# DerekGloudemans/3D-playground

Measured on AMD Instinct MI355X. Metric: training images/sec at 1920x1080, ResNet-50 3D-RetinaNet, higher is better.
Workload: dtype f32; 1 GPU; resnet50 directional 3D-RetinaNet, 1920x1080 synthetic frames, batch 8 per GPU, 10 GT boxes/image, fp32, fwd+loss+bwd+clip+Adam (BASELINE configs[1]); global_batch=8, parallelism=dp1

## Files before the change

3d-playground_amd/retinanet_mi355x/_hip.py:

```python
import ctypes
import os

import torch

_HERE = os.path.dirname(os.path.abspath(__file__))
LIB_PATH = os.environ.get("RN_LIB_PATH") or os.path.join(_HERE, "lib", "libretinanet_mi355x.so")
_lib = None

c_i32, c_i64, c_f32, c_f64, c_vp = ctypes.c_int, ctypes.c_int64, ctypes.c_float, ctypes.c_double, ctypes.c_void_p

SIGNATURES = {
    "rn_version": (ctypes.c_char_p, []),
    "rn_check_device": (c_i32, []),
    "rn_get_fp32_mfma": (c_i32, []),
    "rn_set_fp32_mfma": (c_i32, [c_i32]),
    "rn_get_option": (c_i32, [c_i32]),
    "rn_set_option": (c_i32, [c_i32, c_i32]),
    "rn_fp32_split_min_k": (c_i32, []),
    "rn_split_weights": (c_i32, [c_vp, c_vp, c_i64, c_i32, c_vp]),
    "rn_split_weights_f16": (c_i32, [c_vp, c_vp, c_vp, c_i64, c_i32, c_vp]),
    "rn_amax": (c_i32, [c_vp, c_i64, c_i32, c_vp, c_vp]),
    "rn_stream_capture_id": (c_i32, [c_vp, ctypes.POINTER(ctypes.c_ulonglong)]),
    "rn_anchor_count": (c_i64, [c_i32, c_i32]),
    "rn_anchor_base_boxes": (None, [c_vp]),
# ... 167 lines not shown
    "rn_tile_lists": (c_i32, [c_vp, c_i64, c_vp, c_vp, c_vp, c_vp, c_vp]),
    "rn_wino_input_both_group_lists": (c_i32, [ctypes.POINTER(WinoGroup), c_vp, c_vp, c_i32, c_i64, c_i64, c_vp, c_vp, c_vp, c_vp, c_vp, c_vp]),
    "rn_wino_output_group_flags": (c_i32, [ctypes.POINTER(WinoGroup), c_vp, c_i32, c_i64, c_i64, c_vp, c_vp, c_i32, c_i32, c_i64, c_vp, c_vp, c_vp]),
    "rn_wino_output_group": (c_i32, [ctypes.POINTER(WinoGroup), c_vp, c_i32, c_i64, c_i64, c_vp, c_vp, c_i32, c_i32, c_i64, c_vp]),
    "rn_conv_igemm_grouped": (c_i32, [ctypes.POINTER(ConvGroup), c_vp, c_vp, c_vp, c_vp]),
    "rn_conv_igemm": (c_i32, [ctypes.POINTER(ConvDesc), c_vp, c_vp, c_vp, c_vp, c_vp, c_vp, c_vp, c_vp, c_vp]),
    "rn_conv_splitk_workspace_bytes": (c_i64, [ctypes.POINTER(ConvDesc)]),
    "rn_conv_igemm_wants_f16": (c_i32, [ctypes.POINTER(ConvDesc)]),
    "rn_conv_igemm_splitk": (c_i32, [ctypes.POINTER(ConvDesc)] + [c_vp] * 10),
    "rn_conv_wgrad": (c_i32, [c_vp, c_i32, c_vp, c_vp, c_vp] + [c_i32] * 12 + [c_vp]),
    "rn_pack_weights": (c_i32, [c_vp, c_vp] + [c_i32] * 7 + [c_vp] + [c_i32] * 4 + [c_vp]),
    "rn_unpack_wgrad": (c_i32, [c_vp, c_vp, c_vp] + [c_i32] * 6 + [c_vp] * 7),
    "rn_bn_fold": (c_i32, [c_vp, c_vp, c_vp, c_vp, c_f32, c_i32, c_vp, c_vp, c_vp, c_vp]),
    "rn_nchw_to_nhwc4": (c_i32, [c_vp, c_vp, c_i32, c_i32, c_i32, c_vp, c_vp]),
    "rn_maxpool_fwd": (c_i32, [c_vp, c_vp, c_vp] + [c_i32] * 6 + [c_vp]),
    "rn_maxpool_bwd": (c_i32, [c_vp, c_vp, c_vp, c_vp] + [c_i32] * 7 + [c_vp, c_vp]),
    "rn_colsum": (c_i32, [c_vp, c_i64, c_i32, c_i32, c_vp, c_i32, c_vp, c_vp]),
    "rn_colsum_workspace_bytes": (c_i64, [c_i64, c_i32]),
    "rn_upsample_add_bwd": (c_i32, [c_vp, c_vp] + [c_i32] * 6 + [c_vp, c_vp]),
    "rn_relu_mask": (c_i32, [c_vp, c_vp, c_i64, c_vp]),
    "rn_sigmoid_bwd_pad": (c_i32, [c_vp, c_vp, c_vp, c_i32, c_i64, c_i32, c_i32, c_i64, c_vp, c_vp]),
    "rn_sigmoid_bwd_pad_flags": (c_i32, [c_vp, c_vp, c_vp, c_i32, c_i32, c_i32, c_i32, c_i32, c_i64, c_vp, c_vp, c_vp]),
    "rn_add_inplace": (c_i32, [c_vp, c_vp, c_i64, c_i64, c_vp, c_vp]),
    "rn_wino_input": (c_i32, [c_vp, c_vp, c_i32, c_i32, c_i32, c_i32, c_i64, c_i64, c_vp]),
    "rn_wino_output": (c_i32, [c_vp, c_vp, c_i32, c_i32, c_i32, c_i32, c_i64, c_i64, c_vp, c_vp, c_vp, c_vp, c_i32, c_i32, c_i64, c_vp]),
    "rn_wino_weights": (c_i32, [c_vp, c_vp, c_i32, c_i32, c_i32, c_vp, c_vp]),
    "rn_wino_dy": (c_i32, [c_vp, c_vp, c_i32, c_i32, c_i32, c_i32, c_i64, c_i64, c_vp]),
    "rn_wino_dw": (c_i32, [c_vp, c_vp, c_i32, c_i32, c_vp]),
    "rn_conv_wgrad_batched": (c_i32, [c_vp, c_i32, c_vp, c_vp, c_vp, c_i32, c_i64, c_i64, c_i64, c_i32] + [c_i32] * 12 + [c_vp, c_i32, c_vp, c_i32, c_vp]),
    "rn_conv_wgrad_batched_det": (c_i32, [c_vp, c_i32, c_vp, c_vp, c_vp, c_i32, c_i64, c_i64, c_i64, c_i32] + [c_i32] * 12 + [c_vp, c_i32, c_vp, c_i32, c_vp, c_i64, c_vp]),
    "rn_conv_wgrad_batched_flags": (c_i32, [c_vp, c_i32, c_vp, c_vp, c_vp, c_i32, c_i64, c_i64, c_i64, c_i32] + [c_i32] * 12 + [c_vp, c_i32, c_vp, c_i32, c_vp, c_vp, c_i64, c_vp]),
    "rn_conv_wgrad_det_workspace_bytes": (c_i64, [c_i32, c_i32, c_i64] + [c_i32] * 9),
    "rn_conv_wgrad_plan": (c_i32, [c_i32, c_i32, c_i64, c_i64, c_i64, c_i32] + [c_i32] * 12 + [c_i32, c_i32, c_i32, c_vp]),
    "rn_f32_to_bf16": (c_i32, [c_vp, c_vp, c_i64, c_vp]),
    "rn_bf16_to_f32": (c_i32, [c_vp, c_vp, c_i64, c_vp]),
    "rn_conv_igemm_bf16": (c_i32, [ctypes.POINTER(ConvDesc), c_vp, c_vp, c_vp, c_i32, c_vp, c_vp, c_vp, c_vp, c_vp]),
    "rn_conv_igemm_bf16_grouped": (c_i32, [ctypes.POINTER(ConvGroup), c_vp, c_i32, c_vp, c_vp, c_vp]),
    "rn_conv_igemm_bf16_tile_rows": (c_i32, [ctypes.POINTER(ConvGroup), c_i32]),
    "rn_maxpool_fwd_fp8out": (c_i32, [c_vp, c_vp] + [c_i32] * 6 + [c_f32, c_vp]),
    "rn_conv_igemm_fp8_tile_rows": (c_i32, [ctypes.POINTER(ConvGroup), c_i32]),
    "rn_conv_igemm_fp8_tile": (c_i32, [ctypes.POINTER(ConvDesc), c_i32]),
    "rn_conv_igemm_bf16_tile": (c_i32, [ctypes.POINTER(ConvDesc), c_i32]),
    "rn_fp8_quantize": (c_i32, [c_vp, c_vp, c_i64, c_f32, c_vp]),
    "rn_fp8_dequantize": (c_i32, [c_vp, c_vp, c_i64, c_f32, c_vp]),
    "rn_fp8_to_bf16": (c_i32, [c_vp, c_vp, c_i64, c_f32, c_vp]),
    "rn_bf16_to_fp8": (c_i32, [c_vp, c_vp, c_i64, c_f32, c_vp]),
    "rn_fp8_quantize_rows": (c_i32, [c_vp, c_vp, c_vp, c_i64, c_i32, c_vp]),
    "rn_conv_igemm_fp8": (c_i32, [ctypes.POINTER(ConvDesc), c_vp, c_vp, c_vp, c_i32, c_vp, c_vp, c_vp, c_f32, c_f32, c_vp]),
    "rn_conv_igemm_fp8_grouped": (c_i32, [ctypes.POINTER(ConvGroup), c_vp, c_i32, c_vp, c_vp, c_f32, c_f32, c_vp]),
    "rn_conv_wgrad_bf16": (c_i32, [c_vp, c_i32, c_vp, c_vp, c_vp] + [c_i32] * 11 + [c_vp]),
    "rn_conv_wgrad_bf16_grouped": (c_i32, [c_i32, ctypes.POINTER(c_vp), c_i32, ctypes.POINTER(c_vp), c_vp, c_vp, c_i32,
                                           ctypes.POINTER(c_i32), ctypes.POINTER(c_i32)] + [c_i32] * 6 + [c_vp]),
    "rn_maxpool_fwd_bf16out": (c_i32, [c_vp, c_vp, c_vp] + [c_i32] * 6 + [c_vp]),
    "rn_maxpool_bwd_bf16in": (c_i32, [c_vp, c_vp, c_vp, c_vp] + [c_i32] * 7 + [c_vp]),
    "rn_upsample_add_bwd_bf16": (c_i32, [c_vp, c_vp] + [c_i32] * 6 + [c_vp]),
    "rn_sigmoid_bwd_pad_bf16": (c_i32, [c_vp, c_vp, c_vp, c_i32, c_i64, c_i32, c_i32, c_i64, c_vp]),
    "rn_relu_bf16": (c_i32, [c_vp, c_vp, c_i64, c_vp]),
    "rn_opt_workspace_bytes": (c_i64, [c_i32]),
    "rn_opt_clip_adam": (c_i32, [c_vp, c_vp, c_i32, c_f32, c_f32, c_f32, c_f32, c_f32, c_i32, c_i32, c_vp, c_vp, c_vp]),
    "rn_opt_clip_adam_dev": (c_i32, [c_vp, c_vp, c_i32, c_f32, c_f32, c_f32, c_f32, c_f32, c_vp, c_i32, c_vp, c_vp, c_vp]),
    "rn_opt_clip_adam_hp": (c_i32, [c_vp, c_vp, c_i32, c_vp, c_vp, c_i32, c_vp, c_vp, c_vp]),
})


RN_ERRORS = {10001: "RN_EINVAL (bad size / unsupported shape)",
             10002: "RN_ETOOMANY (more than RN_MAX_GT=256 label rows per image)"}
# ... 51 lines not shown
```

3d-playground_amd/retinanet_mi355x/conv.py:

```python
import ctypes
import os

import torch

from . import _hip, prof

ConvDesc = _hip.ConvDesc

ACT_NONE, ACT_RELU, ACT_SIGMOID = 0, 1, 2


def kpad(kh, kw, c):
    return (kh * kw * c + 31) // 32 * 32


def out_size(n, k, stride, pad):
    return (n + 2 * pad - k) // stride + 1


def pack_weights(weight, mode=0, scale=None, kw_pad=None, c_pad=None, taps=None, presplit=True):
    lib = _hip.load()
    w = _hip.f32c(weight.detach())
    _hip.need_gpu(w, scale)
    cout, cin, kh, kw = w.shape
# ... 653 lines not shown
def dgrad_s2_classes(dy, class_weights, in_hw, cin, k, pad, flops=0.0, **kw):
    N, Ho, Wo, _ = dy.shape
    Hi, Wi = in_hw
    dx = torch.empty((N, Hi, Wi, cin), dtype=torch.float32, device=dy.device)
    classes = s2_classes(k, pad)
    if len(classes) < 4:
        dx.zero_()
    total_taps = sum(c[2][1] * c[2][3] for c in classes)
    slot = amax_slot(dy.device, N) if want_amax() else None
    for (ph, pw, (r0, nr, s0, ns), (dh0, dw0)), wc in zip(classes, class_weights):
        gh, gw = (Hi - ph + 1) // 2, (Wi - pw + 1) // 2
        if gh <= 0 or gw <= 0:
            continue
        conv_igemm(dy, wc, dx, (gh, gw, cin, nr, ns, 1, -1, (dh0, dw0), 0), out_map=(2, ph, pw, Hi, Wi),
                   flops=flops * nr * ns / total_taps, amax=slot, **kw)
    if slot is not None:
        amax_attach(dx, slot)
    return dx


def wgrad(dy, x, dw, cout, k, stride, pad, kw_pad=None, in_relu=False, flops=0.0, colsum=None):
    lib = _hip.load()
    N, Ho, Wo, ldy = dy.shape
    _, Hi, Wi, Cin = x.shape
    kind = "conv_wgrad" + (" %dx%dx%d %d->%d k%d s%d" % (N, Ho, Wo, Cin, cout, k, stride) if prof.BY_SHAPE else "")
    am = (amax_words(dy), amax_words(x)) if want_amax() and dy.is_contiguous() and x.is_contiguous() else (None, None)
    rc = prof.timed(kind, flops, lambda: _wgrad_call(
        lib, dy.device, dy.data_ptr(), ldy, x.data_ptr(), dw.data_ptr(), _hip.ptr(colsum), 1, 0, 0, 0, 0,
        (N, Hi, Wi, Cin, Ho, Wo, cout, k, k if kw_pad is None else kw_pad, stride, pad, int(in_relu)), amax=am))
    _hip.check(rc, "rn_conv_wgrad")
    return dw


def unpack_wgrad(dw, w_packed, weight_shape, kw_pad=None, c_pad=None, scale=None, mean=None, rstd=None, colsum=None,
                 want_bn=False, out=None):
    lib = _hip.load()
    cout, cin, kh, kw = weight_shape
    kw_pad = kw if kw_pad is None else kw_pad
    c_pad = (cin + 3) // 4 * 4 if c_pad is None else c_pad
    if out is not None:
        dweight, dgamma, dbeta = out
        assert tuple(dweight.shape) == tuple(weight_shape) and dweight.is_contiguous() and dweight.dtype == torch.float32
        assert (dgamma is not None) == bool(want_bn) and (dbeta is not None) == (colsum is not None)
    else:
        dweight = torch.empty(weight_shape, dtype=torch.float32, device=dw.device)
        dgamma = torch.empty(cout, dtype=torch.float32, device=dw.device) if want_bn else None
        dbeta = torch.empty(cout, dtype=torch.float32, device=dw.device) if colsum is not None else None
    _hip.check(lib.rn_unpack_wgrad(dw.data_ptr(), _hip.ptr(w_packed), dweight.data_ptr(), cout, cin, kh, kw, kw_pad,
                                   c_pad, _hip.ptr(scale), _hip.ptr(mean), _hip.ptr(rstd), _hip.ptr(colsum),
                                   _hip.ptr(dgamma), _hip.ptr(dbeta), _hip.stream()), "rn_unpack_wgrad")
    return dweight, dgamma, dbeta


def bn_fold(gamma, beta, mean, var, eps=1e-5):
    lib = _hip.load()
    C = gamma.numel()
    out = torch.empty((3, C), dtype=torch.float32, device=gamma.device)
    _hip.check(lib.rn_bn_fold(_hip.f32c(gamma.detach()).data_ptr(), _hip.f32c(beta.detach()).data_ptr(),
                              _hip.f32c(mean).data_ptr(), _hip.f32c(var).data_ptr(), eps, C, out[0].data_ptr(),
                              out[1].data_ptr(), out[2].data_ptr(), _hip.stream()), "rn_bn_fold")
    return out[0], out[1], out[2]


def nchw_to_nhwc4(img):
    lib = _hip.load()
    img = _hip.f32c(img)
# ... 398 lines not shown
```

3d-playground_amd/retinanet_mi355x/engine.py:

```python
import os

import torch

from . import _hip, arch, conv as cv, ops, prof


FUSE_DY = os.environ.get("RN_WINO_FUSE_DY", "1") != "0"
SPARSE_REG = os.environ.get("RN_SPARSE_REG", "1") != "0"
SPARSE_REG_LISTS = os.environ.get("RN_SPARSE_REG_LISTS", "1") != "0"
GROUPED_WGRAD_BF16 = os.environ.get("RN_GROUPED_WGRAD_BF16", "1") != "0"
S2_SHORTCUT_COMPACT = os.environ.get("RN_S2_SHORTCUT_COMPACT", "1") != "0"
STEM_BF16_PRODUCTS = os.environ.get("RN_STEM_BF16_PRODUCTS", "1") != "0"


def _qscale(t):
    return getattr(t, "_rn_scale", None) or getattr(t, "_rn_qscale", None)


def _as_fp8(t):
    if t is None or t.dtype == torch.uint8:
        return t
    q = getattr(t, "_rn_q8", None)
    if q is None:
        sc = _qscale(t)
# ... 311 lines not shown
            return
        for g, x in zip(gs, xs):
            self.bwd_params(g, x)

    def bwd_data(self, g, in_hw, add=None, mask=None, mask_mode=2, add2=None):
        s = self.spec
        if self.bf16:
            assert add2 is None
            kw = dict(add=add, add_mode=1 if add is not None else 0, mask=mask, mask_mode=mask_mode,
                      flops=self.flops(g.shape[0], g.shape[1], g.shape[2]))
            if s.stride == 2 and s.k > 1:
                return cv.dgrad_s2_classes_bf16(g, self.dgrad_weights16(), in_hw, s.cin, s.k, s.pad, **kw)
            if s.stride == 2 and s.k == 1 and s.pad == 0 and mask is None and S2_SHORTCUT_COMPACT:
                Hi, Wi = in_hw
                N, Ho, Wo, _ = g.shape
                if add is None:
                    dx = torch.zeros((N, Hi, Wi, s.cin), dtype=torch.bfloat16, device=g.device)
                else:
                    assert add.shape == (N, Hi, Wi, s.cin) and add.dtype == torch.bfloat16 and add.is_contiguous()
                    dx = add
                return cv.conv_igemm_bf16(g, self.dgrad_weights16(), dx, (Ho, Wo, s.cin, 1, 1, 1, -1, 0, 0), out_map=(2, 0, 0, Hi, Wi),
                                          add=add, add_mode=1 if add is not None else 0, flops=kw["flops"])
            return cv.dgrad_any_bf16(g, self.dgrad_weights16(), in_hw, s.cin, s.k, s.stride, s.pad, **kw)
        if self.wino_active and add2 is None and g.shape[3] == s.cout and g.is_contiguous():
            ready, self.dy_v = getattr(self, "dy_v", None), None
            return cv.wino_conv_group([g], self.wino_weights(1), adds=None if add is None else [add],
                                      masks=None if mask is None else [mask], mask_mode=mask_mode, V_ready=ready)[0]
        kw = dict(add=add, add_mode=1 if add is not None else 0, mask=mask, mask_mode=mask_mode,
                  flops=self.flops(g.shape[0], g.shape[1], g.shape[2]))
        if s.stride == 2 and s.k > 1:
            assert add2 is None
            return cv.dgrad_s2_classes(g, self.dgrad_weights(), in_hw, s.cin, s.k, s.pad, **kw)
        return cv.dgrad(g, self.dgrad_weights(), in_hw, s.cin, s.k, s.stride, s.pad, add2=add2, **kw)

    def bwd_data_compact(self, g):
        s = self.spec
        assert s.k == 1 and s.stride == 2
        N, Ho, Wo, _ = g.shape
        out = torch.empty((N, Ho, Wo, s.cin), dtype=torch.float32, device=g.device)
        return cv.conv_igemm(g, self.dgrad_weights(), out, (Ho, Wo, s.cin, 1, 1, 1, -1, 0, 0), flops=self.flops(N, Ho, Wo))

    def grad_names(self):
        s = self.spec
        if s.bn:
            return [s.name + ".weight", s.bn + ".weight", s.bn + ".bias"]
        return [s.name + ".weight"] + ([s.name + ".bias"] if s.bias else [])

    def finish(self, out=None):
        s = self.spec
        dst = None
        if out is not None:
            names = self.grad_names()
            dst = (out[names[0]], out[names[1]] if s.bn else None, out[names[-1]] if len(names) > 1 else None)
        dweight, dgamma, dbeta = cv.unpack_wgrad(
            self.dw, self.wf, tuple(self.weight.shape), kw_pad=self.kw_pad, c_pad=self.cin_pad, scale=self.scale,
            mean=self.mean, rstd=self.rstd, colsum=self.cs, want_bn=bool(s.bn), out=dst)
        out = {s.name + ".weight": dweight}
        if s.bn:
            out[s.bn + ".weight"] = dgamma
            out[s.bn + ".bias"] = dbeta
        elif s.bias:
            out[s.name + ".bias"] = dbeta
        self.dw = self.cs = self.wd = self.uf = self.ud = self.saved_v = self.dy_v = None
        return out


# ... 567 lines not shown
                main0.wait_stream(ws)
                cv.side_release(ws)
            held.clear()

        def aside(fn, tensors):
            nonlocal wg_count
            ws = wss[wg_count % len(wss)]
            wg_count += 1
            if cv.want_amax():
                for t in tensors:
                    if t.dtype == torch.float32 and t.is_contiguous():
                        cv.amax_words(t)
            ws.wait_event(torch.cuda.current_stream(dreg.device).record_event())
            with torch.cuda.stream(ws):
                fn()
            held.append(tuple(tensors) + tuple(getattr(t, "_rn_amax", (None,))[0] for t in tensors))

        def wg(L, g, x, in_relu=False):
            if wss is None:
                L.bwd_params(g, x, in_relu=in_relu)
            elif L.wino_active and not L.bf16:
                L.bwd_params(g, x, in_relu=in_relu, side=wss[0] if os.environ.get("RN_WGRAD_WINO", "1") != "0" else None)
            else:
                aside(lambda: L.bwd_params(g, x, in_relu=in_relu), (g, x))

        def wg_group(L, gs, xs, wino=False, flags=None, lists=None):
            if wss is None or os.environ.get("RN_WGRAD_TOWERS", "0") == "0":
                L.bwd_params_group(gs, xs, wino=wino, flags=flags, lists=lists)
            elif wino or L.wino_active:
                L.bwd_params_group(gs, xs, wino=wino, side=wss[0], flags=flags, lists=lists)
            else:
                aside(lambda: L.bwd_params_group(gs, xs), tuple(gs) + tuple(xs))

        def done(layer):
            nonlocal next_bucket
            if batched:
                pending.append(layer)
                grads.update({n: views[n] for n in layer.grad_names()})
            else:
                g = layer.finish(views)
                grads.update(g)
                if self.grad_hook is not None:
                    self.grad_hook(g)
            if flat is not None and layer.spec.name == buckets[next_bucket][2]:
                if batched:
                    join()
                    self._unpack_bucket(next_bucket, pending, views)
                    pending.clear()
                if self.bucket_hook is not None:
                    self.bucket_hook(next_bucket, flat[buckets[next_bucket][0]:buckets[next_bucket][1]])
                next_bucket += 1

        ACT = _as_bf16 if self.fp8 else (lambda t: t)
        pyramid, counts = [ACT(t) for t in S["pyramid"]], S["counts"]
        B = dreg.shape[0]
        A = dreg.shape[1]
        dpyr = [None] * 5
        hws = [(f.shape[1], f.shape[2]) for f in pyramid]
        side = self.tower_streams(dreg.device)
        main = torch.cuda.current_stream(dreg.device)
        if side is not None:
            fork = main.record_event()
        retired = []
        for ti, (prefix, dout, width, sig) in enumerate((("regressionModel", dreg, self.n_reg, None),
                                                         ("classificationModel", dcls, self.num_classes, cls))):
            Lout = Ls[prefix + ".output"]
# ... 59 lines not shown
        done(L)
        L = Ls["fpn.P3_1"]
        wg(L, dp3sum, c3)
        dc3 = L.bwd_data(dp3sum, hw(c3))
        done(L)
        L = Ls["fpn.P4_2"]
        wg(L, dp4, p4sum)
        dp4sum = L.bwd_data(dp4, hw(p4sum))
        cv.upsample_add_bwd(dp3sum, dp4sum)
        done(L)
        L = Ls["fpn.P4_1"]
        wg(L, dp4sum, c4)
        dc4 = L.bwd_data(dp4sum, hw(c4))
        done(L)
        L = Ls["fpn.P5_2"]
        wg(L, dp5, p5lat)
        dp5lat = L.bwd_data(dp5, hw(p5lat))
        cv.upsample_add_bwd(dp4sum, dp5lat)
        done(L)
        L = Ls["fpn.P5_1"]
        wg(L, dp5lat, c5)
        dc5 = L.bwd_data(dp5lat, hw(c5), add=dc5, mask=c5)
        done(L)
        lateral = {"layer2": dc3, "layer3": dc4}
        g = dc5
        nblocks = len(self.blocks)
        for bi in range(nblocks - 1, -1, -1):
            pre, roles = self.blocks[bi]
            xin, t1, t2, z = (ACT(t) for t in S["blocks"][bi])
            S["blocks"][bi] = None
            in_hw = hw(xin)
            last = roles["conv2"] if self.kind == "basic" else roles["conv3"]
            tin = t1 if self.kind == "basic" else t2
            wg(last, g, tin)
            gt = last.bwd_data(g, hw(tin), mask=tin)
            done(last)
            if self.kind != "basic":
                wg(roles["conv2"], gt, t1)
                gt = roles["conv2"].bwd_data(gt, hw(t1), mask=t1)
                done(roles["conv2"])
            layer_name = pre.split(".")[0]
            first_of_layer = pre.endswith(".0")
            extra = None
            if first_of_layer and bi > 0:
                prev_layer = self.blocks[bi - 1][0].split(".")[0]
                extra = lateral.get(prev_layer)
            dcompact = None
            if "down" in roles:
                wg(roles["down"], g, xin)
                if roles["down"].spec.stride == 2 and roles["conv1"].spec.stride == 1 and not self.bwd16:
                    dcompact = roles["down"].bwd_data_compact(g)
                    dres = extra
                else:
                    dres = roles["down"].bwd_data(g, in_hw, add=extra)
                done(roles["down"])
            else:
                dres = g if extra is None else cv.add_(extra, g)
            wg(roles["conv1"], gt, xin)
            g = roles["conv1"].bwd_data(gt, in_hw, add=dres, mask=xin if bi > 0 else None, add2=dcompact)
            done(roles["conv1"])
            del layer_name
        gstem = (cv.maxpool_bwd_bf16 if self.bwd16 else cv.maxpool_bwd)(S["stem"], g, S["pool_arg"], relu_mask=True)
        wg(Ls["conv1"], gstem, S["x4"])
        done(Ls["conv1"])
        join()
        assert flat is None or next_bucket == len(buckets), "backward finished layers in an order finish_order() does not describe"
        return grads
```

include/retinanet_mi355x.h:

```cpp
#ifndef RETINANET_MI355X_H
#define RETINANET_MI355X_H

#include <stdint.h>

#ifdef __cplusplus
extern "C" {
#endif

#define RN_OK 0
#define RN_EINVAL 10001
#define RN_ETOOMANY 10002
#define RN_MAX_GT 256
#define RN_LEVELS 5

const char *rn_version(void);
int rn_check_device(void);

int64_t rn_anchor_count(int height, int width);
void rn_anchor_base_boxes(double out[RN_LEVELS * 9 * 4]);
int rn_anchors_fwd(float *out, int height, int width, void *stream);

int rn_pairwise_iou(const float *a, const float *b, float *iou, int64_t A, int N, void *stream);

int64_t rn_focal_workspace_bytes(int B, int64_t A);
// ... 246 lines not shown
typedef struct rn_conv_group {
    int n;
    int tile_end[RN_MAX_GROUP];
    rn_conv_desc d[RN_MAX_GROUP];
    const float *x[RN_MAX_GROUP];
    float *y[RN_MAX_GROUP];
    const float *add[RN_MAX_GROUP];
    const float *mask[RN_MAX_GROUP];
} rn_conv_group;
int rn_conv_igemm_grouped(const rn_conv_group *g, const float *w_packed, const float *scale, const float *shift,
                          void *stream);

int rn_conv_wgrad(const float *dy, int ldy, const float *x, float *dw, float *colsum, int N, int Hi, int Wi,
                  int Cin, int Ho, int Wo, int Cout, int kh, int kw, int stride, int pad, int in_relu, void *stream);
int rn_conv_wgrad_batched(const float *dy, int ldy, const float *x, float *dw, float *colsum, int nbatch,
                          int64_t dy_bstride, int64_t x_bstride, int64_t dw_bstride, int colsum_batch, int N, int Hi, int Wi,
                          int Cin, int Ho, int Wo, int Cout, int kh, int kw, int stride, int pad, int in_relu,
                          const void *dy_amax, int dy_amax_n, const void *x_amax, int x_amax_n, void *stream);
int64_t rn_conv_wgrad_det_workspace_bytes(int ldy, int nbatch, int64_t dw_bstride, int N, int Hi, int Wi, int Cin, int Ho, int Wo,
                                          int Cout, int kh, int kw);
int rn_conv_wgrad_batched_det(const float *dy, int ldy, const float *x, float *dw, float *colsum, int nbatch,
                              int64_t dy_bstride, int64_t x_bstride, int64_t dw_bstride, int colsum_batch, int N, int Hi, int Wi,
                              int Cin, int Ho, int Wo, int Cout, int kh, int kw, int stride, int pad, int in_relu,
                              const void *dy_amax, int dy_amax_n, const void *x_amax, int x_amax_n, void *workspace, int64_t workspace_bytes,
                              void *stream);
int rn_conv_wgrad_batched_flags(const float *dy, int ldy, const float *x, float *dw, float *colsum, int nbatch,
                                int64_t dy_bstride, int64_t x_bstride, int64_t dw_bstride, int colsum_batch, int N, int Hi, int Wi,
                                int Cin, int Ho, int Wo, int Cout, int kh, int kw, int stride, int pad, int in_relu,
                                const void *dy_amax, int dy_amax_n, const void *x_amax, int x_amax_n, const void *k_active,
                                void *workspace, int64_t workspace_bytes, void *stream);
int rn_conv_wgrad_plan(int ldy, int nbatch, int64_t dy_bstride, int64_t x_bstride, int64_t dw_bstride, int colsum_batch, int N, int Hi,
                       int Wi, int Cin, int Ho, int Wo, int Cout, int kh, int kw, int stride, int pad, int in_relu, int have_amax,
                       int have_flags, int det, int32_t *out);

int rn_f32_to_bf16(const float *src, void *dst, int64_t n, void *stream);
int rn_bf16_to_f32(const void *src, float *dst, int64_t n, void *stream);
int rn_conv_igemm_bf16(const rn_conv_desc *d, const void *x, const void *w_packed, void *y, int y_is_f32,
                       const float *scale, const float *shift, const void *add, const void *mask, void *stream);
int rn_conv_igemm_bf16_grouped(const rn_conv_group *g, const void *w_packed, int y_is_f32, const float *scale,
                               const float *shift, void *stream);
int rn_conv_igemm_bf16_tile_rows(const rn_conv_group *g, int y_is_f32);
int rn_fp8_quantize(const float *src, void *dst, int64_t n, float inv_scale, void *stream);
int rn_maxpool_fwd_fp8out(const float *x, void *y, int N, int H, int W, int C, int Ho, int Wo, float inv_scale, void *stream);
int rn_fp8_dequantize(const void *src, float *dst, int64_t n, float scale, void *stream);
int rn_fp8_to_bf16(const void *src, void *dst, int64_t n, float scale, void *stream);
int rn_bf16_to_fp8(const void *src, void *dst, int64_t n, float inv_scale, void *stream);
int rn_fp8_quantize_rows(const float *w_packed, void *w_q, float *row_scale, int64_t rows, int Kpad, void *stream);
int rn_conv_igemm_fp8(const rn_conv_desc *d, const void *x_q, const void *w_q, void *y, int y_is_f32, const float *scale,
                      const float *shift, const void *add_q, float add_scale, float out_inv_scale, void *stream);
int rn_conv_igemm_fp8_tile_rows(const rn_conv_group *g, int y_is_f32);
int rn_conv_igemm_fp8_tile(const rn_conv_desc *d, int y_is_f32);
int rn_conv_igemm_bf16_tile(const rn_conv_desc *d, int y_is_f32);
int rn_conv_igemm_fp8_grouped(const rn_conv_group *g, const void *w_q, int y_is_f32, const float *scale, const float *shift,
                              float add_scale, float out_inv_scale, void *stream);

int rn_conv_wgrad_bf16(const void *dy, int ldy, const void *x, float *dw, float *colsum, int N, int Hi, int Wi, int Cin,
                       int Ho, int Wo, int Cout, int kh, int kw, int stride, int pad, void *stream);
int rn_conv_wgrad_bf16_grouped(int n, const void *const *dy, int ldy, const void *const *x, float *dw, float *colsum, int N,
                               const int *Hi, const int *Wi, int Cin, int Cout, int kh, int kw, int stride, int pad, void *stream);

int rn_maxpool_fwd_bf16out(const float *x, void *y, uint8_t *argmax, int N, int H, int W, int C, int Ho, int Wo, void *stream);
int rn_maxpool_bwd_bf16in(const float *x, const void *dy, const uint8_t *argmax, float *dx, int N, int H, int W, int C, int Ho,
                          int Wo, int relu_mask, void *stream);
int rn_upsample_add_bwd_bf16(const void *src, void *dst, int N, int Hs, int Ws, int Hd, int Wd, int C, void *stream);
int rn_sigmoid_bwd_pad_bf16(const float *dy, const float *s, void *out, int B, int64_t rows_per_image, int C, int ld,
                            int64_t src_batch_stride, void *stream);
// ... 343 lines not shown
```

Baseline: 132.6 images/sec.

## Fuse 1x1 conv weight-gradient and data-gradient into one backward kernel for 64->256

Adds a HIP kernel that computes both dW and dX for 1x1 stride-1 convolutions with Cin=64, Cout=256 in a single pass. Each dy tile is loaded once, split into fp16 hi/lo operands in LDS, and used for both the split-precision MFMA weight-gradient accumulation and the data-gradient product. The kernel also folds in the column sum, the ReLU mask and the amax tracking. This removes the second read of dy and one launch per bottleneck conv3 and downsample layer of that shape. In exchange it accumulates dw with global atomicAdd, so results are non-deterministic; it is gated off in deterministic mode.

```diff
diff --git a/3d-playground_amd/csrc/conv_bwd_1x1.hip b/3d-playground_amd/csrc/conv_bwd_1x1.hip
--- /dev/null
+++ b/3d-playground_amd/csrc/conv_bwd_1x1.hip
@@ -0,0 +1,283 @@
+#include <type_traits>
+
+#include "common.h"
+#include "conv_bwd_1x1_geom.h"
+#include "mfma_split.h"
+
+#if !RN_EXPERIMENT
+#undef RN_BF_KO
+#endif
+#ifndef RN_BF_KO
+#define RN_BF_KO 0
+#endif
+#if !RN_EXPERIMENT
+#undef RN_BF_ND
+#endif
+#ifndef RN_BF_ND
+#define RN_BF_ND 1
+#endif
+
+typedef float f32x16 __attribute__((ext_vector_type(16)));
+typedef float f32x4v __attribute__((ext_vector_type(4)));
+typedef short s16x4w __attribute__((ext_vector_type(4)));
+typedef short s16x8w __attribute__((ext_vector_type(8)));
+
+struct Bwd1x1Args {
+    const float *dy, *x;
+    const char *wd;
+    const float *w_unscale;
+    float *dx, *dw, *colsum;
+    const void *mask;
+    unsigned *sign_out;
+    const void *dy_amax, *x_amax;
+    void *dx_amax;
+    int HW, spi, per;
+};
+
+__device__ __forceinline__ f16x8 bf_tr_operand(const char *img, unsigned a0, unsigned a1) {
+    typedef __attribute__((address_space(3))) s16x4w *lp;
+    const s16x4w lo = __builtin_amdgcn_ds_read_tr16_b64_v4i16((lp)(__attribute__((address_space(3))) char *)(img + a0));
+    const s16x4w hi = __builtin_amdgcn_ds_read_tr16_b64_v4i16((lp)(__attribute__((address_space(3))) char *)(img + a1));
+    const s16x8w v = {lo[0], lo[1], lo[2], lo[3], hi[0], hi[1], hi[2], hi[3]};
+    return __builtin_bit_cast(f16x8, v);
+}
+
+template <int MASK>
+__global__ __launch_bounds__(256, 2) void conv_bwd_1x1_kernel(const Bwd1x1Args p) {
+    using G = Bwd1x1Geom;
+    __shared__ __attribute__((aligned(16))) char lds[2 * G::BUF];
+    __shared__ __attribute__((aligned(16))) char stage[2 * G::STAGE];
+    static_assert(4 * G::CO * 4 <= G::BUF, "the column-sum reduction fits a buffer");
+
+    const int tid = threadIdx.x, lane = tid & 63, wave = tid >> 6;
+    const int n = (int)(blockIdx.x / (unsigned)p.spi), slice = (int)blockIdx.x - n * p.spi;
+    const int k0 = slice * p.per;
+    const int npx = (k0 + p.per < p.HW ? k0 + p.per : p.HW) - k0;
+    if (npx <= 0) return;
+    const int nks = (npx + G::WK - 1) / G::WK;
+    const int64_t pix0 = (int64_t)n * p.HW + k0;
+    const __amdgpu_buffer_rsrc_t rs_dy = __builtin_amdgcn_make_buffer_rsrc(const_cast<float *>(p.dy + pix0 * G::CO), (short)0,
+                                                                           (int)((unsigned)npx * (unsigned)(G::CO * 4)), 0x00020000);
+    const __amdgpu_buffer_rsrc_t rs_x = __builtin_amdgcn_make_buffer_rsrc(const_cast<float *>(p.x + pix0 * G::CI), (short)0,
+                                                                          (int)((unsigned)npx * (unsigned)(G::CI * 4)), 0x00020000);
+    const int se_dy = rn_f16_scale_exp_of(rn_amax_exp(p.dy_amax, n)), se_x = rn_f16_scale_exp_of(rn_amax_exp(p.x_amax, n));
+    const float s_dy = rn_exp_to_float(se_dy), u_dy = rn_exp_to_float(254 - se_dy);
+    const float s_x = rn_exp_to_float(se_x), u_x = rn_exp_to_float(254 - se_x);
+
+    f16x8 wh[8], wl[8];
+    {
+        const char *wrow = p.wd + (16 * wave + (lane & 15)) * (G::CO * 4) + (lane >> 5) * 64 + ((lane >> 4) & 1) * 16;
+#pragma unroll
+        for (int kb = 0; kb < 8; ++kb) {
+            wh[kb] = *reinterpret_cast<const f16x8 *>(wrow + kb * 128);
+            wl[kb] = *reinterpret_cast<const f16x8 *>(wrow + kb * 128 + 32);
+        }
+    }
+    __shared__ __attribute__((aligned(16))) float wus[G::CI];
+    if (tid < G::CI) wus[tid] = p.w_unscale[tid];
+
+    struct Regs { f32x4v a[4], b; };
+    const unsigned dy_voff = (unsigned)(((tid >> 6) * G::CO + 4 * lane) * 4);
+    const unsigned x_voff = (unsigned)(tid * 16);
+    auto load_step = [&](int ks, Regs &r) {
+        const unsigned so = (unsigned)ks * (unsigned)(G::WK * G::CO * 4);
+#pragma unroll
+        for (int i = 0; i < 4; ++i)
+            r.a[i] = __builtin_bit_cast(f32x4v, __builtin_amdgcn_raw_buffer_load_b128(rs_dy, (int)(dy_voff + i * (4 * G::CO * 4)), (int)so, 0));
+        r.b = __builtin_bit_cast(f32x4v, __builtin_amdgcn_raw_buffer_load_b128(rs_x, (int)x_voff, (int)((unsigned)ks * (unsigned)(G::WK * G::CI * 4)), 0));
+    };
+    unsigned wr_dy[4];
+#pragma unroll
+    for (int i = 0; i < 4; ++i) wr_dy[i] = (unsigned)G::dy_wr(tid, i);
+    const unsigned wr_x = (unsigned)G::x_wr(tid);
+    float cs4[4] = {0.f, 0.f, 0.f, 0.f};
+    auto split_store = [&](int buf, const Regs &r) {
+        char *B = &lds[buf * G::BUF];
+#pragma unroll
+        for (int i = 0; i < 4; ++i) {
+            unsigned h[2], l[2];
+#pragma unroll
+            for (int j = 0; j < 4; ++j) cs4[j] += r.a[i][j];
+            split_pair_h(r.a[i][0], r.a[i][1], s_dy, h[0], l[0]);
+            split_pair_h(r.a[i][2], r.a[i][3], s_dy, h[1], l[1]);
+            *reinterpret_cast<uint2 *>(B + wr_dy[i]) = make_uint2(h[0], h[1]);
+            *reinterpret_cast<uint2 *>(B + G::DY_IMG + wr_dy[i]) = make_uint2(l[0], l[1]);
+        }
+        unsigned h[2], l[2];
+        split_pair_h(r.b[0], r.b[1], s_x, h[0], l[0]);
+        split_pair_h(r.b[2], r.b[3], s_x, h[1], l[1]);
+        *reinterpret_cast<uint2 *>(B + 2 * G::DY_IMG + wr_x) = make_uint2(h[0], h[1]);
+        *reinterpret_cast<uint2 *>(B + 2 * G::DY_IMG + G::X_IMG + wr_x) = make_uint2(l[0], l[1]);
+    };
+
+    const int e_px = tid >> 4;
+    float *dx_s = p.dx + pix0 * G::CI;
+    unsigned *sign_s = p.sign_out != nullptr ? p.sign_out + pix0 * (G::CI / 32) : nullptr;
+    const float *maskf_s = reinterpret_cast<const float *>(p.mask) + (MASK == 1 ? pix0 * G::CI : 0);
+    const unsigned *maskb_s = reinterpret_cast<const unsigned *>(p.mask) + (MASK == 2 ? pix0 * (G::CI / 32) : 0);
+    struct MaskF { float4 q; };
+    struct MaskB { unsigned w; };
+    typedef typename std::conditional<MASK == 1, MaskF, MaskB>::type MaskT;
+    auto mask_load = [&](int ks) -> MaskT {
+        MaskT m;
+        const int off = ks * (G::WK * G::CI) + 4 * tid;
+        const bool in = ks * G::WK + e_px < npx;
+        if constexpr (MASK == 1) m.q = in ? *reinterpret_cast<const float4 *>(maskf_s + off) : make_float4(0.f, 0.f, 0.f, 0.f);
+        else if constexpr (MASK == 2) m.w = in ? maskb_s[off >> 5] : 0u;
+        else m.w = 0u;
+        return m;
+    };
+    float am = 0.f;
+    const unsigned st_rd = (unsigned)G::st_rd(tid);
+    auto dx_store = [&](int ks, int sbuf, const MaskT mk) {
+        const float4 t = *reinterpret_cast<const float4 *>(&stage[sbuf * G::STAGE + st_rd]);
+        const float4 wu = *reinterpret_cast<const float4 *>(&wus[4 * (tid & 15)]);
+        if (ks * G::WK + e_px < npx) {
+            float v[4] = {t.x * u_dy * wu.x, t.y * u_dy * wu.y, t.z * u_dy * wu.z, t.w * u_dy * wu.w};
+            const int off = ks * (G::WK * G::CI) + 4 * tid;
+            if constexpr (MASK == 1) {
+                const float m[4] = {mk.q.x, mk.q.y, mk.q.z, mk.q.w};
+#pragma unroll
+                for (int j = 0; j < 4; ++j) v[j] = m[j] > 0.f ? v[j] : 0.f;
+            } else if constexpr (MASK == 2) {
+                const unsigned nib = mk.w >> ((unsigned)off & 28u);
+#pragma unroll
+                for (int j = 0; j < 4; ++j) v[j] = (nib >> j) & 1u ? v[j] : 0.f;
+            }
+#if !(RN_BF_KO & 1)
+            *reinterpret_cast<float4 *>(dx_s + off) = make_float4(v[0], v[1], v[2], v[3]);
+#endif
+            if (sign_s != nullptr) rn_sign_store(sign_s, off, v[0], v[1], v[2], v[3]);
+            am = fmaxf(am, fmaxf(fmaxf(fabsf(v[0]), fabsf(v[1])), fmaxf(fabsf(v[2]), fabsf(v[3]))));
+        }
+    };
+
+    unsigned fa[2][2], fb[2][2];
+#pragma unroll
+    for (int t = 0; t < 2; ++t)
+#pragma unroll
+        for (int rd = 0; rd < 2; ++rd) {
+            fa[t][rd] = (unsigned)G::dy_tr(wave, t, rd, lane);
+            fb[t][rd] = (unsigned)(2 * G::DY_IMG + G::x_tr(t, rd, lane));
+        }
+    const unsigned da0 = (unsigned)G::dy_a(lane, 0);
+    unsigned st_wr[4];
+#pragma unroll
+    for (int r = 0; r < 4; ++r) st_wr[r] = (unsigned)G::st_wr(wave, lane, r);
+
+    f32x16 acc[2][2];
+#pragma unroll
+    for (int i = 0; i < 2; ++i)
+#pragma unroll
+        for (int j = 0; j < 2; ++j)
+#pragma unroll
+            for (int e_ = 0; e_ < 16; ++e_) acc[i][j][e_] = 0.f;
+
+    Regs r0, r1;
+    load_step(0, r0);
+    split_store(0, r0);
+    load_step(1, r0);
+    MaskT mk = mask_load(0);
+    __syncthreads();
+    auto k_step = [&](int ks, int buf, Regs &cur, Regs &nxt) {
+        const char *S = &lds[buf * G::BUF];
+        SplitH8 sa[2], sb[2];
+#pragma unroll
+        for (int t = 0; t < 2; ++t) {
+            sa[t].h = bf_tr_operand(S, fa[t][0], fa[t][1]);
+            sa[t].l = bf_tr_operand(S + G::DY_IMG, fa[t][0], fa[t][1]);
+            sb[t].h = bf_tr_operand(S, fb[t][0], fb[t][1]);
+            sb[t].l = bf_tr_operand(S + G::X_IMG, fb[t][0], fb[t][1]);
+        }
+        const MaskT mk_next = mask_load(ks);
+        if (ks > 0) dx_store(ks - 1, buf ^ 1, mk);
+        mk = mk_next;
+        f32x4v dd[RN_BF_ND];
+#pragma unroll
+        for (int c = 0; c < RN_BF_ND; ++c) dd[c] = f32x4v{0.f, 0.f, 0.f, 0.f};
+#if !(RN_BF_KO & 4)
+#pragma unroll
+        for (int kb = 0; kb < 8; ++kb) {
+            const f16x8 ah = *reinterpret_cast<const f16x8 *>(S + (da0 ^ (unsigned)(kb << 6)));
+            const f16x8 al = *reinterpret_cast<const f16x8 *>(S + G::DY_IMG + (da0 ^ (unsigned)(kb << 6)));
+            f32x4v &d = dd[kb % RN_BF_ND];
+            d = __builtin_amdgcn_mfma_f32_16x16x32_f16(al, wh[kb], d, 0, 0, 0);
+            d = __builtin_amdgcn_mfma_f32_16x16x32_f16(ah, wl[kb], d, 0, 0, 0);
+            d = __builtin_amdgcn_mfma_f32_16x16x32_f16(ah, wh[kb], d, 0, 0, 0);
+        }
+#endif
+        f32x4v d = dd[0];
+#pragma unroll
+        for (int c = 1; c < RN_BF_ND; ++c) d += dd[c];
+        split_store(buf ^ 1, cur);
+        load_step(ks + 2, nxt);
+#pragma unroll
+        for (int tm = 0; tm < 2; ++tm)
+#pragma unroll
+            for (int tn = 0; tn < 2; ++tn) RN_SPLITH_MFMA(acc[tm][tn], sa[tm], sb[tn]);
+#pragma unroll
+        for (int r = 0; r < 4; ++r) *reinterpret_cast<float *>(&stage[buf * G::STAGE + st_wr[r]]) = d[r];
+        __syncthreads();
+    };
+    for (int ks = 0; ks < nks; ks += 2) {
+        k_step(ks, 0, r0, r1);
+        if (ks + 1 < nks) k_step(ks + 1, 1, r1, r0);
+    }
+    dx_store(nks - 1, (nks - 1) & 1, mk);
+    rn_amax_note(p.dx_amax, n, am);
+
+    if (p.colsum != nullptr) {
+        float (*csred)[G::CO] = reinterpret_cast<float (*)[G::CO]>(&lds[0]);
+#pragma unroll
+        for (int j = 0; j < 4; ++j) csred[wave][4 * lane + j] = cs4[j];
+        __syncthreads();
+        atomicAdd(p.colsum + tid, csred[0][tid] + csred[1][tid] + csred[2][tid] + csred[3][tid]);
+    }
+    const float us = u_dy * u_x;
+#pragma unroll
+    for (int tm = 0; tm < 2; ++tm)
+#pragma unroll
+        for (int tn = 0; tn < 2; ++tn) {
+            const int col = tn * 32 + (lane & 31);
+#pragma unroll
+            for (int e = 0; e < 16; ++e) {
+                const int row = wave * 64 + tm * 32 + (e & 3) + 8 * (e >> 2) + 4 * (lane >> 5);
+#if RN_BF_KO & 2
+                if (acc[tm][tn][e] == 1.2345e-30f)
+#endif
+                atomicAdd(p.dw + row * G::CI + col, acc[tm][tn][e] * us);
+            }
+        }
+}
+
+extern "C" int rn_conv_bwd_1x1(const float *dy, const float *x, const void *w_split, const float *w_unscale, float *dx, float *dw,
+                               float *colsum, const void *mask, int mask_mode, const float *add, void *sign_out, const void *dy_amax,
+                               const void *x_amax, void *dx_amax, int N, int H, int W, int Cin, int Cout, int stride, void *stream) {
+    using G = Bwd1x1Geom;
+    if (Cin != G::CI || Cout != G::CO || stride != 1 || add != nullptr) return RN_EINVAL;
+    if (rn_get_fp32_mfma() != RN_FP32_SPLIT3 || rn_get_option(RN_OPT_DETERMINISTIC) != 0) return RN_EINVAL;
+    if (!dy || !x || !w_split || !w_unscale || !dx || !dw || !dy_amax || !x_amax) return RN_EINVAL;
+    if (mask_mode < 0 || mask_mode > 2 || (mask_mode != 0) != (mask != nullptr)) return RN_EINVAL;
+    if (N <= 0 || H <= 0 || W <= 0 || N > 65535 || (int64_t)H * W > 0x7fffffff / 64) return RN_EINVAL;
+    if ((((uintptr_t)dy | (uintptr_t)x | (uintptr_t)dx | (uintptr_t)w_split) & 15) || (((uintptr_t)dw | (uintptr_t)colsum | (uintptr_t)w_unscale) & 3))
+        return RN_EINVAL;
+    if (((uintptr_t)mask & (mask_mode == 1 ? 15 : 3)) || ((uintptr_t)sign_out & 3)) return RN_EINVAL;
+    Bwd1x1Args a;
+    a.dy = dy; a.x = x; a.wd = reinterpret_cast<const char *>(w_split); a.w_unscale = w_unscale;
+    a.dx = dx; a.dw = dw; a.colsum = colsum; a.mask = mask; a.sign_out = reinterpret_cast<unsigned *>(sign_out);
+    a.dy_amax = dy_amax; a.x_amax = x_amax; a.dx_amax = dx_amax;
+    a.HW = H * W;
+    static const int wgs = rn_env_int("RN_BWD_FUSED_WGS", 1536);
+    int spi = wgs / N < 1 ? 1 : wgs / N;
+    int per = ((a.HW + spi - 1) / spi + G::WK - 1) / G::WK * G::WK;
+    if (per < 128) per = 128;
+    if (per > (1 << 20)) per = 1 << 20;
+    a.per = per;
+    a.spi = (a.HW + per - 1) / per;
+    const dim3 grid((unsigned)(a.spi * N));
+    if (mask_mode == 0) hipLaunchKernelGGL(conv_bwd_1x1_kernel<0>, grid, dim3(256), 0, (hipStream_t)stream, a);
+    else if (mask_mode == 1) hipLaunchKernelGGL(conv_bwd_1x1_kernel<1>, grid, dim3(256), 0, (hipStream_t)stream, a);
+    else hipLaunchKernelGGL(conv_bwd_1x1_kernel<2>, grid, dim3(256), 0, (hipStream_t)stream, a);
+    RN_LAUNCH_CHECK();
+    return RN_OK;
+}
diff --git a/3d-playground_amd/csrc/conv_bwd_1x1_geom.h b/3d-playground_amd/csrc/conv_bwd_1x1_geom.h
--- /dev/null
+++ b/3d-playground_amd/csrc/conv_bwd_1x1_geom.h
@@ -0,0 +1,46 @@
+#pragma once
+
+#ifdef __HIPCC__
+#define RN_HD __host__ __device__ __forceinline__
+#else
+#define RN_HD inline
+#endif
+
+struct Bwd1x1Geom {
+    static constexpr int CO = 256, CI = 64, WK = 16;
+    static constexpr int DY_ROWB = 2 * CO, X_ROWB = 2 * CI;
+    static constexpr int DY_IMG = WK * DY_ROWB, X_IMG = WK * X_ROWB;
+    static constexpr int BUF = 2 * DY_IMG + 2 * X_IMG;
+    static constexpr int ST_LD = CI + 4;
+    static constexpr int STAGE = WK * ST_LD * 4;
+    static RN_HD int swd(int row) { return ((row & 3) << 2) | ((0x1320 >> (4 * (row >> 2))) & 3); }
+    static RN_HD int swx(int row) { return 4 * ((row >> 1) & 1); }
+    static RN_HD int dy_pixel(int tid, int i) { return (tid >> 6) + 4 * i; }
+    static RN_HD int x_pixel(int tid) { return tid >> 4; }
+    static RN_HD int dy_wr(int tid, int i) {
+        const int row = dy_pixel(tid, i), l = tid & 63;
+        return DY_ROWB * row + 16 * ((l >> 1) ^ swd(row)) + 8 * (l & 1);
+    }
+    static RN_HD int x_wr(int tid) {
+        const int row = x_pixel(tid), c4 = tid & 15;
+        return X_ROWB * row + 16 * ((c4 >> 1) ^ swx(row)) + 8 * (c4 & 1);
+    }
+    static RN_HD int dy_tr(int wave, int t, int rd, int lane) {
+        const int g = lane >> 4, q = (lane & 15) >> 2, pp = lane & 3;
+        const int row = 8 * (g >> 1) + 4 * rd + q;
+        const int ch = (64 * wave + 32 * t + 16 * (g & 1)) / 8 + (pp >> 1);
+        return DY_ROWB * row + 16 * (ch ^ swd(row)) + 8 * (pp & 1);
+    }
+    static RN_HD int x_tr(int t, int rd, int lane) {
+        const int g = lane >> 4, q = (lane & 15) >> 2, pp = lane & 3;
+        const int row = 8 * (g >> 1) + 4 * rd + q;
+        const int ch = (32 * t + 16 * (g & 1)) / 8 + (pp >> 1);
+        return X_ROWB * row + 16 * (ch ^ swx(row)) + 8 * (pp & 1);
+    }
+    static RN_HD int dy_a(int lane, int kb) {
+        const int row = lane & 15;
+        return DY_ROWB * row + 16 * ((4 * kb + (lane >> 4)) ^ swd(row));
+    }
+    static RN_HD int st_wr(int wave, int lane, int r) { return ((4 * (lane >> 4) + r) * ST_LD + 16 * wave + (lane & 15)) * 4; }
+    static RN_HD int st_rd(int tid) { return ((tid >> 4) * ST_LD + 4 * (tid & 15)) * 4; }
+};
diff --git a/3d-playground_amd/retinanet_mi355x/_hip.py b/3d-playground_amd/retinanet_mi355x/_hip.py
--- a/3d-playground_amd/retinanet_mi355x/_hip.py
+++ b/3d-playground_amd/retinanet_mi355x/_hip.py
@@ -223,6 +223,7 @@
     "rn_conv_wgrad_batched_flags": (c_i32, [c_vp, c_i32, c_vp, c_vp, c_vp, c_i32, c_i64, c_i64, c_i64, c_i32] + [c_i32] * 12 + [c_vp, c_i32, c_vp, c_i32, c_vp, c_vp, c_i64, c_vp]),
     "rn_conv_wgrad_det_workspace_bytes": (c_i64, [c_i32, c_i32, c_i64] + [c_i32] * 9),
     "rn_conv_wgrad_plan": (c_i32, [c_i32, c_i32, c_i64, c_i64, c_i64, c_i32] + [c_i32] * 12 + [c_i32, c_i32, c_i32, c_vp]),
+    "rn_conv_bwd_1x1": (c_i32, [c_vp] * 8 + [c_i32] + [c_vp] * 5 + [c_i32] * 6 + [c_vp]),
     "rn_f32_to_bf16": (c_i32, [c_vp, c_vp, c_i64, c_vp]),
     "rn_bf16_to_f32": (c_i32, [c_vp, c_vp, c_i64, c_vp]),
     "rn_conv_igemm_bf16": (c_i32, [ctypes.POINTER(ConvDesc), c_vp, c_vp, c_vp, c_i32, c_vp, c_vp, c_vp, c_vp, c_vp]),
diff --git a/3d-playground_amd/retinanet_mi355x/conv.py b/3d-playground_amd/retinanet_mi355x/conv.py
--- a/3d-playground_amd/retinanet_mi355x/conv.py
+++ b/3d-playground_amd/retinanet_mi355x/conv.py
@@ -709,6 +709,47 @@
     return dw
 
 
+BWD_FUSED_1X1 = os.environ.get("RN_BWD_FUSED_1X1", "1") != "0"
+BWD_FUSED_SHAPES = frozenset({(64, 256)})
+BWD_FUSED_LAUNCHES = 0
+
+
+def bwd_1x1_fused(dy, x, w_dgrad, dw, colsum, mask=None, mask_mode=None, flops=0.0, sign=False):
+    global BWD_FUSED_LAUNCHES
+    lib = _hip.load()
+    N, H, W, cout = dy.shape
+    cin = x.shape[3]
+    tw = getattr(w_dgrad, "_rn_split16", None)
+    if tw is None:
+        raise RuntimeError("bwd_1x1_fused needs the fp16 twin of the data-gradient weights (split3 mode)")
+    if not (dy.is_contiguous() and x.is_contiguous() and dy.dtype == x.dtype == torch.float32 and x.shape[:3] == dy.shape[:3]):
+        raise RuntimeError("bwd_1x1_fused: dy and x must be dense fp32 tensors over the same pixels")
+    mptr, mmode = None, 0
+    if mask is not None:
+        bits = getattr(mask, "_rn_sign", None)
+        if mask_mode is None:
+            mask_mode = 2 if (bits is not None and BITMASKS) else 1
+        if mask_mode == 2 and bits is None:
+            raise RuntimeError("bwd_1x1_fused: mask_mode 2 needs a mask that carries its sign bits")
+        mptr, mmode = (bits if mask_mode == 2 else mask).data_ptr(), mask_mode
+    dy_am, x_am = amax_words(dy), amax_words(x)
+    dx = torch.empty((N, H, W, cin), dtype=torch.float32, device=dy.device)
+    sbits = _sign_words(dx, sign)
+    dx_am = amax_slot(dy.device, N)
+    kind = "conv_bwd_fused" + (" %dx%dx%d %d->%d" % (N, H, W, cin, cout) if prof.BY_SHAPE else "")
+    nb = 0.0
+    if prof.ACTIVE is not None:
+        nb = 4.0 * (dy.numel() + x.numel() + dx.numel() * (1 + {0: 0.0, 1: 1.0, 2: 1.0 / 32}[mmode] + (1.0 / 32 if sbits is not None else 0.0))
+                    + w_dgrad.numel() + dw.numel() + cout)
+    rc = prof.timed(kind, 2.0 * flops, lambda: lib.rn_conv_bwd_1x1(
+        dy.data_ptr(), x.data_ptr(), tw[0].data_ptr(), tw[1].data_ptr(), dx.data_ptr(), dw.data_ptr(), _hip.ptr(colsum), mptr, mmode,
+        None, _hip.ptr(sbits), dy_am.data_ptr(), x_am.data_ptr(), dx_am.data_ptr(), N, H, W, cin, cout, 1, _hip.stream()), nb)
+    _hip.check(rc, "rn_conv_bwd_1x1")
+    BWD_FUSED_LAUNCHES += 1
+    amax_attach(dx, dx_am)
+    return dx
+
+
 def unpack_wgrad(dw, w_packed, weight_shape, kw_pad=None, c_pad=None, scale=None, mean=None, rstd=None, colsum=None,
                  want_bn=False, out=None):
     lib = _hip.load()
diff --git a/3d-playground_amd/retinanet_mi355x/engine.py b/3d-playground_amd/retinanet_mi355x/engine.py
--- a/3d-playground_amd/retinanet_mi355x/engine.py
+++ b/3d-playground_amd/retinanet_mi355x/engine.py
@@ -367,6 +367,21 @@
             assert add2 is None
             return cv.dgrad_s2_classes(g, self.dgrad_weights(), in_hw, s.cin, s.k, s.pad, **kw)
         return cv.dgrad(g, self.dgrad_weights(), in_hw, s.cin, s.k, s.stride, s.pad, add2=add2, **kw)
+
+    def bwd_fused_ok(self, g, x):
+        s = self.spec
+        return (not self.bf16 and not self.fp8 and s.k == 1 and s.stride == 1 and s.pad == 0 and (s.cin, s.cout) in cv.BWD_FUSED_SHAPES
+                and g.dtype == torch.float32 and x.dtype == torch.float32 and g.is_contiguous() and x.is_contiguous()
+                and g.shape[3] == s.cout and x.shape[3] == s.cin and x.shape[:3] == g.shape[:3]
+                and cv.get_fp32_mfma() == "split3" and cv.want_amax() and not cv.get_option(cv.OPT_DETERMINISTIC)
+                and getattr(self.dgrad_weights(), "_rn_split16", None) is not None)
+
+    def bwd_fused(self, g, x, mask=None):
+        s = self.spec
+        if self.dw is None:
+            self.dw = torch.zeros_like(self.wf)
+            self.cs = torch.zeros(s.cout, dtype=torch.float32, device=g.device)
+        return cv.bwd_1x1_fused(g, x, self.dgrad_weights(), self.dw, self.cs, mask=mask, flops=self.flops(g.shape[0], g.shape[1], g.shape[2]))
 
     def bwd_data_compact(self, g):
         s = self.spec
@@ -1000,6 +1015,9 @@
             else:
                 aside(lambda: L.bwd_params_group(gs, xs), tuple(gs) + tuple(xs))
 
+        def fused(L, g, x):
+            return cv.BWD_FUSED_1X1 and not self.bwd16 and not self.fp8 and self.grad_hook is None and L.bwd_fused_ok(g, x)
+
         def done(layer):
             nonlocal next_bucket
             if batched:
@@ -1125,8 +1143,11 @@
             in_hw = hw(xin)
             last = roles["conv2"] if self.kind == "basic" else roles["conv3"]
             tin = t1 if self.kind == "basic" else t2
-            wg(last, g, tin)
-            gt = last.bwd_data(g, hw(tin), mask=tin)
+            if fused(last, g, tin):
+                gt = last.bwd_fused(g, tin, mask=tin)
+            else:
+                wg(last, g, tin)
+                gt = last.bwd_data(g, hw(tin), mask=tin)
             done(last)
             if self.kind != "basic":
                 wg(roles["conv2"], gt, t1)
@@ -1140,11 +1161,14 @@
                 extra = lateral.get(prev_layer)
             dcompact = None
             if "down" in roles:
-                wg(roles["down"], g, xin)
-                if roles["down"].spec.stride == 2 and roles["conv1"].spec.stride == 1 and not self.bwd16:
+                if extra is None and fused(roles["down"], g, xin):
+                    dres = roles["down"].bwd_fused(g, xin)
+                elif roles["down"].spec.stride == 2 and roles["conv1"].spec.stride == 1 and not self.bwd16:
+                    wg(roles["down"], g, xin)
                     dcompact = roles["down"].bwd_data_compact(g)
                     dres = extra
                 else:
+                    wg(roles["down"], g, xin)
                     dres = roles["down"].bwd_data(g, in_hw, add=extra)
                 done(roles["down"])
             else:
diff --git a/include/retinanet_mi355x.h b/include/retinanet_mi355x.h
--- a/include/retinanet_mi355x.h
+++ b/include/retinanet_mi355x.h
@@ -302,6 +302,9 @@
 int rn_conv_wgrad_plan(int ldy, int nbatch, int64_t dy_bstride, int64_t x_bstride, int64_t dw_bstride, int colsum_batch, int N, int Hi,
                        int Wi, int Cin, int Ho, int Wo, int Cout, int kh, int kw, int stride, int pad, int in_relu, int have_amax,
                        int have_flags, int det, int32_t *out);
+int rn_conv_bwd_1x1(const float *dy, const float *x, const void *w_split, const float *w_unscale, float *dx, float *dw, float *colsum,
+                    const void *mask, int mask_mode, const float *add, void *sign_out, const void *dy_amax, const void *x_amax,
+                    void *dx_amax, int N, int H, int W, int Cin, int Cout, int stride, void *stream);
 
 int rn_f32_to_bf16(const float *src, void *dst, int64_t n, void *stream);
 int rn_bf16_to_f32(const void *src, float *dst, int64_t n, void *stream);
```

After: 133.9 images/sec (median of 6 runs). +1.0%, better.
